# rslmtoasa/rslmtoasa

Measured on AMD Instinct MI355X. Metric: block-recursion throughput (H|psi> + A_n + B_n recursion levels, recursion.f90 recur_b), higher is better.
Workload: dtype f64

## Files before the change

### rslmtoasa_amd/csrc/kernels_mfma.hpp

```cpp
#pragma once
#include <hip/hip_runtime.h>
#include <string>
#include <vector>
#include "kernels_valu.hpp"

namespace rsrec {

typedef double double4_t __attribute__((ext_vector_type(4)));

constexpr int GROUP = 8;
constexpr int MF_WAVES = 4;

struct LayoutCI {
    static __device__ __forceinline__ double2 ld(const double* b, int r, int c) { return make_double2(b[36 * r + 2 * c], b[36 * r + 2 * c + 1]); }
    static __device__ __forceinline__ void st(double* b, int r, int c, double2 v) { b[36 * r + 2 * c] = v.x; b[36 * r + 2 * c + 1] = v.y; }
};
__host__ __device__ constexpr int gram_col(int part, int c, int ci) { return ci ? 2 * c + part : 18 * part + c; }

__device__ __forceinline__ int active_workgroups(int ngroups) { return max(1, min((int)gridDim.x, (ngroups + MF_WAVES - 1) / MF_WAVES)); }

struct GroupWalk {
    int g, end, step;
    __device__ __forceinline__ GroupWalk(int ngroups, int wave, int nbx_eff = 0) {
        const int nbx = nbx_eff > 0 ? nbx_eff : gridDim.x, bx = blockIdx.x;
        const int xcd = bx & 7, j = bx >> 3;
        const int per_xcd = (nbx >> 3) + ((xcd < (nbx & 7)) ? 1 : 0);
        const int chunk = (ngroups + 7) >> 3;
        const int lo = xcd * chunk;
        end = min(ngroups, lo + chunk);
        g = lo + j * MF_WAVES + wave;
        step = per_xcd * MF_WAVES;
        if (nbx < 8) { g = bx * MF_WAVES + wave; end = ngroups; step = nbx * MF_WAVES; }
    }
};


struct RowRef { unsigned off; bool valid; };
__device__ __forceinline__ RowRef group_row(const int* __restrict__ grp, int rho, int zero_block) {
    const int slot = rho / 18, r = rho - 18 * slot;
    const int a = grp[slot];
    RowRef R;
    R.valid = a >= 0;
    R.off = (unsigned)BLD * (unsigned)(R.valid ? a : zero_block) + 36u * (unsigned)r;
    return R;
}

struct GramAcc {
    double4_t t00, t01, t10, t11;
    double tr0, tr1;
    double t0r, t1r;
    double trr;
    __device__ __forceinline__ void zero() { t00 = t01 = t10 = t11 = (double4_t){0, 0, 0, 0}; tr0 = tr1 = t0r = t1r = trr = 0.0; }
    __device__ __forceinline__ void to_lds(double* G , int lane, bool sym) const {
        const int l15 = lane & 15, l4 = lane >> 4, l3 = lane & 3, lg = (lane >> 2) & 3;
#pragma unroll
        for (int j = 0; j < 4; ++j) {
            const int r = l4 + 4 * j;
            G[36 * r + l15] = t00[j];
            G[36 * r + 16 + l15] = t01[j];
            G[36 * (16 + r) + 16 + l15] = t11[j];
            if (!sym) G[36 * (16 + r) + l15] = t10[j];
        }
        G[36 * (32 + l4) + l15] = tr0;
        G[36 * (32 + l4) + 16 + l15] = tr1;
        if (!sym) { G[36 * (4 * lg + l4) + 32 + l3] = t0r; G[36 * (16 + 4 * lg + l4) + 32 + l3] = t1r; }
        if (lg == 0) G[36 * (32 + l4) + 32 + l3] = trr;
    }
};

__device__ __forceinline__ void gram_block_out(const GramAcc& A, double* lds , double* gout , bool sym) {
    const int lane = threadIdx.x & 63, wave = threadIdx.x >> 6;
    A.to_lds(lds + wave * 1296, lane, sym);
    __syncthreads();
    for (int e = threadIdx.x; e < 1296; e += blockDim.x) {
        double s = 0.0;
#pragma unroll
        for (int wv = 0; wv < MF_WAVES; ++wv) s += lds[wv * 1296 + e];
        if (sym) {
            const int r = e / 36, c = e % 36;
            const bool have = (r >= 32) || (r < 16) || (c >= 16 && c < 32);
            if (!have || (r < 32 && c >= 32)) {
                double t = 0.0;
#pragma unroll
                for (int wv = 0; wv < MF_WAVES; ++wv) t += lds[wv * 1296 + 36 * c + r];
                s = t;
            }
        }
        gout[e] = s;
    }
}

#ifndef RSREC_NT_STREAMS
#define RSREC_NT_STREAMS 0
#endif
template <class T> __device__ __forceinline__ T ld_stream(const T* p) {
#if RSREC_NT_STREAMS
    return __builtin_nontemporal_load(p);
#else
    return *p;
#endif
}
__device__ __forceinline__ double2 ld_stream(const double2* p) {
#if RSREC_NT_STREAMS
    typedef double nt_d2 __attribute__((ext_vector_type(2)));
    const nt_d2 v = __builtin_nontemporal_load(reinterpret_cast<const nt_d2*>(p));
    return make_double2(v[0], v[1]);
#else
    return *p;
#endif
}
template <class T> __device__ __forceinline__ void st_stream(T* p, T v) {
#if RSREC_NT_STREAMS
    __builtin_nontemporal_store(v, p);
#else
    *p = v;
#endif
}

constexpr int S5_GRAM_DOUBLES = 584;
constexpr long S5_GRAM_MIN_NEVER = 1L << 40;
constexpr int S5_GRAM_MAXW = 8;
__host__ __device__ inline bool s5_gram_folds(long ngroups, long min_groups) { return ngroups > 0 && ngroups >= min_groups; }
__host__ __device__ inline int s5_gram_workgroups(int ngroups) { return ngroups / 4 < 1 ? 1 : (ngroups / 4 < S5_GRAM_MAXW ? ngroups / 4 : S5_GRAM_MAXW); }
struct GramFold { const int* cum = nullptr; int nlev = 0; long min_groups = 0; };

__global__ __launch_bounds__(640) void k_gram_groupsum(GramFold F, int level, const double* __restrict__ gpart, size_t cstride, double* __restrict__ partial ) {
    __shared__ double sm[S5_GRAM_DOUBLES];
    const int chain = blockIdx.y, w = blockIdx.x;
    const int ngroups = F.cum[(size_t)chain * F.nlev + level] / GROUP;
    if (!s5_gram_folds(ngroups, F.min_groups)) return;
    double* img = partial + ((size_t)chain * gridDim.x + w) * 1296;
    const int nw = s5_gram_workgroups(ngroups);
    if (w >= nw) {
        for (int e = threadIdx.x; e < 1296; e += blockDim.x) img[e] = 0.0;
        return;
    }
    const size_t g0 = (size_t)w * ngroups / nw, g1 = (size_t)(w + 1) * ngroups / nw;
    if (threadIdx.x < S5_GRAM_DOUBLES) {
        const double* src = gpart + (size_t)chain * cstride + threadIdx.x;
        double s = 0.0;
        size_t q = 2 * g0;
        for (; q + 16 <= 2 * g1; q += 16) {
            double v[16];
#pragma unroll
            for (int i = 0; i < 16; ++i) v[i] = ld_stream(src + (q + i) * S5_GRAM_DOUBLES);
#pragma unroll
            for (int i = 0; i < 16; ++i) s += v[i];
        }
        for (; q < 2 * g1; ++q) s += ld_stream(src + q * S5_GRAM_DOUBLES);
        sm[threadIdx.x] = s;
    }
    __syncthreads();
    for (int e = threadIdx.x; e < 1296; e += blockDim.x) {
        const int r = e / 36, c = e - 36 * r, a = r >> 1, b = c >> 1, part = c & 1;
        double v = 0.0;
        if ((r & 1) == 0) {
            if (a < 16 && b < 16) v = sm[256 * part + 4 * (16 * (a & 3) + b) + (a >> 2)];
            else if (a >= 16 && b < 16) v = sm[512 + 2 * (16 * (a - 16) + b) + part];
            else if (a >= 16) v = sm[576 + 2 * (2 * (a - 16) + (b - 16)) + part];
            else { const double t = sm[512 + 2 * (16 * (b - 16) + a) + part]; v = part ? -t : t; }
        }
        img[e] = v;
    }
}

#ifndef ADOT_UNROLL
#define ADOT_UNROLL 4
#endif
__global__ __launch_bounds__(MF_WAVES * 64, 2) void k_mfma_adot(ChainView CV, int level, int zero_block, const double* __restrict__ psi,
                                                               const double* __restrict__ tvec, double* partial ,
                                                               GramFold F = GramFold() ) {
    __shared__ double lds[MF_WAVES * 1296];
    const int chain = blockIdx.y;
    if (F.cum && s5_gram_folds(F.cum[(size_t)chain * F.nlev + level] / GROUP, F.min_groups)) return;
    const int lane = threadIdx.x & 63;
    const int wave = __builtin_amdgcn_readfirstlane(threadIdx.x >> 6);
    const int ngroups = CV.count_of(chain, level) / GROUP;
    const int* order = CV.order_of(chain, level);
    const size_t vo = (size_t)chain * CV.vstride;
    const double* ps = psi + vo;
    const double* tv = tvec + vo;
    const int l15 = lane & 15, l4 = lane >> 4, l3 = lane & 3;
    GramAcc A;
    A.zero();
    const int nbx = active_workgroups(ngroups);
    for (GroupWalk w((int)blockIdx.x < nbx ? ngroups : 0, wave, nbx); w.g < w.end; w.g += w.step) {
        const int* grp = order + (size_t)w.g * GROUP;
#pragma unroll ADOT_UNROLL
        for (int kq = 0; kq < 36; ++kq) {
            const RowRef rk = group_row(grp, 4 * kq + l4, zero_block);
            const double p0 = ld_stream(ps + rk.off + l15), p1 = ld_stream(ps + rk.off + 16 + l15), pr = ld_stream(ps + rk.off + 32 + l3);
            const double h0 = ld_stream(tv + rk.off + l15), h1 = ld_stream(tv + rk.off + 16 + l15), hr = ld_stream(tv + rk.off + 32 + l3);
            A.t00 = __builtin_amdgcn_mfma_f64_16x16x4f64(p0, h0, A.t00, 0, 0, 0);
            A.t01 = __builtin_amdgcn_mfma_f64_16x16x4f64(p0, h1, A.t01, 0, 0, 0);
            A.t10 = __builtin_amdgcn_mfma_f64_16x16x4f64(p1, h0, A.t10, 0, 0, 0);
            A.t11 = __builtin_amdgcn_mfma_f64_16x16x4f64(p1, h1, A.t11, 0, 0, 0);
            A.tr0 = __builtin_amdgcn_mfma_f64_4x4x4f64(pr, h0, A.tr0, 0, 0, 0);
            A.tr1 = __builtin_amdgcn_mfma_f64_4x4x4f64(pr, h1, A.tr1, 0, 0, 0);
            A.t0r = __builtin_amdgcn_mfma_f64_4x4x4f64(p0, hr, A.t0r, 0, 0, 0);
            A.t1r = __builtin_amdgcn_mfma_f64_4x4x4f64(p1, hr, A.t1r, 0, 0, 0);
            A.trr = __builtin_amdgcn_mfma_f64_4x4x4f64(pr, hr, A.trr, 0, 0, 0);
        }
    }
    gram_block_out(A, lds, partial + ((size_t)chain * gridDim.x + blockIdx.x) * 1296, false);
}

struct SpmmDims {
    int kk, nslots, nmax, nlev, cpo, ostride, level; size_t vstride; const int* obase; int nchains = 0;
    int sat_base = 0, run_lo = 0, run_hi = 0, nskip = 0, skip_lo[4] = {0, 0, 0, 0}, skip_hi[4] = {0, 0, 0, 0};
    int nruns = 0, run_tau[4] = {0, 0, 0, 0}, run_glo[4] = {0, 0, 0, 0}, run_ghi[4] = {0, 0, 0, 0}, run_row0[5] = {0, 0, 0, 0, 0};
    int skip_pa = 0;
};

__device__ __forceinline__ double2 reduce_gram(const double* __restrict__ partial , int nblk, double* lds , int ci = 0) {
    for (int e = threadIdx.x; e < 1296; e += blockDim.x) {
        double s = 0.0;
        for (int p = 0; p < nblk; ++p) s += partial[(size_t)p * 1296 + e];
        lds[e] = s;
    }
    __syncthreads();
    double2 c = make_double2(0, 0);
    if (threadIdx.x < BLK) {
        const int cp = threadIdx.x % NB, cc = threadIdx.x / NB;
        const int rp = gram_col(0, cp, ci), ip = gram_col(1, cp, ci), rc = gram_col(0, cc, ci), ic = gram_col(1, cc, ci);
        c.x = lds[36 * rp + rc] + lds[36 * ip + ic];
        c.y = lds[36 * rp + ic] - lds[36 * ip + rc];
    }
    __syncthreads();
    return c;
}

}
```

### rslmtoasa_amd/csrc/kernels_spmm5.hpp

```cpp
#pragma once
#include <hip/hip_runtime.h>
#include <algorithm>
#include <type_traits>
#include <utility>
#include <vector>
#include "kernels_valu.hpp"
#include "kernels_mfma.hpp"
#include "kernels_spmm4.hpp"

namespace rsrec {

#ifndef RSREC_S5_KSPLIT_PROBE
#define RSREC_S5_KSPLIT_PROBE 0
#endif
#ifndef RSREC_S5_PRIO
#define RSREC_S5_PRIO 0
#endif
#ifndef RSREC_S5_GRAM_STRIP_LOADS
#define RSREC_S5_GRAM_STRIP_LOADS 0
#endif
#ifndef S5_WG_GROUPS
#define S5_WG_GROUPS 4
#endif
constexpr int S5_TRIPLE = 640;
// ... 744 lines not shown
                        ecr[i] = cb[eo[i] + 288 + (l4 & 1)];
                    }
                    if (epi.kind == 2) {
                        const double* zb = epi.old + vo;
#pragma unroll
                        for (int i = 0; i < 3; ++i) {
#pragma unroll
                            for (int p = 0; p < 2; ++p) ez[i][p] = *reinterpret_cast<const s5_d2*>(zb + eo[i] + 36 * (4 * p + l4));
                            ezr[i] = zb[eo[i] + 288 + (l4 & 1)];
                        }
                    }
                }
#pragma unroll
                for (int i = 0; i < 3; ++i) {
                    const int a = av[i];
                    double* ob = out + eo[i];
#pragma unroll
                    for (int p = 0; p < 2; ++p) {
                        s5_d2 v; v[0] = acc3.m[i][2 * p]; v[1] = acc3.m[i][2 * p + 1];
                        if (epi.kind) {
                            v[0] = (v[0] - epi.b * ec[i][p][0]) / epi.a; v[1] = (v[1] - epi.b * ec[i][p][1]) / epi.a;
                            if (epi.kind == 2) { v[0] = v[0] * 2.0 - ez[i][p][0]; v[1] = v[1] * 2.0 - ez[i][p][1]; }
                        }
                        if (a != zero_block) *reinterpret_cast<s5_d2*>(ob + 36 * (4 * p + l4)) = v;
                    }
                    double r = acc3.r[i];
                    if (epi.kind) {
                        r = (r - epi.b * ecr[i]) / epi.a;
                        if (epi.kind == 2) r = r * 2.0 - ezr[i];
                    }
                    if (a != zero_block && l4 < 2) ob[288 + l4] = r;
                }
            };
            int ratom[GROUP];
            if (part < 2) {
                int a3[3];
#pragma unroll
                for (int j = 0; j < 3; ++j) { const int a = grp[3 * part + j]; a3[j] = a >= 0 ? a : zero_block; }
#pragma unroll
                for (int t = 0; t < GROUP; ++t) ratom[t] = zero_block;
                s5_run_stream_n<TWO, 3, false>(acc3, M3, fr3, inb, in2b, nbr, a3, ratom, 0, ncol, sig, l4, lane_main, lane_z, lane_rem, lane_rem_z, lane16, lane8);
                finish3(std::false_type{}, a3);
            } else {
#pragma unroll
                for (int t = 0; t < GROUP; ++t) { const int a = grp[t]; ratom[t] = a >= 0 ? a : zero_block; }
                const int a2[2] = {ratom[6], ratom[7]};
                int mra = grp[l15 >> 1];
                mra = mra >= 0 ? mra : zero_block;
                s5_run_stream_n<TWO, 2, true>(acc3, M3, fr3, inb, in2b, nbr, a2, ratom, l15 >> 1, ncol, sig, l4, lane_main, lane_z, lane_rem, lane_rem_z, lane16, lane8);
                const int av[3] = {a2[0], a2[1], mra};
                finish3(std::true_type{}, av);
            }
            continue;
        }
        int atom[GROUP];
        int vatom[GROUP], tile_blk[GROUP];
        int my_rem_atom, rem_blk = 0;
        if constexpr (OCT) {
            const int a0 = g;
#pragma unroll
            for (int t = 0; t < GROUP; ++t) {
                const bool ok = a0 >= 0 && chain + t < D.nchains;
                atom[t] = ok ? a0 : zero_block;
                tile_blk[t] = ok ? t * (D.kk + 1) : 0;
                vatom[t] = ok ? a0 + t * (D.kk + 1) : zero_block;
            }
            const int tr = l15 >> 1;
            const bool okr = a0 >= 0 && chain + tr < D.nchains;
            rem_blk = okr ? tr * (D.kk + 1) : 0;
            my_rem_atom = okr ? a0 + tr * (D.kk + 1) : zero_block;
        } else {
#pragma unroll
            for (int t = 0; t < GROUP; ++t) { const int a = grp[t]; atom[t] = a >= 0 ? a : zero_block; vatom[t] = atom[t]; tile_blk[t] = 0; }
            my_rem_atom = grp[l15 >> 1];
            my_rem_atom = my_rem_atom >= 0 ? my_rem_atom : zero_block;
        }
        const int first = atom[0];
        if (!OCT && D.skip_pa && first < D.nmax) continue;
        const int tau = first < D.nmax ? first : D.nmax + izp[first];
        const int* __restrict__ M = meta + (size_t)tau * Spmm5Operator::META;
        const char* __restrict__ fr = LDSA ? reinterpret_cast<const char*>(s5_lds) : reinterpret_cast<const char*>(frag + ((size_t)tau * 2 + sig) * ntr * S5_TRIPLE);
        const char* __restrict__ fh = (TWO && frag_head) ? reinterpret_cast<const char*>(frag_head + ((size_t)chain * ntau + tau) * S5_HEAD_DOUBLES + (size_t)sig * S5_HEAD_TRIPLES * S5_TRIPLE) : nullptr;

        S5Acc acc;
#pragma unroll
        for (int t = 0; t < 9; ++t) { acc.m[t] = (double4_t){0, 0, 0, 0}; acc.r[t] = 0.0; }

        if constexpr (OCT) s5_run_stream<TWO, LDSA, true>(acc, M, fr, fh, inb, in2b, nbr, atom, l15 >> 1, ncol, sig, l4, lane_main, lane_z, lane_rem, lane_rem_z, lane16, lane8, tile_blk, rem_blk);
        else s5_run_stream<TWO, LDSA>(acc, M, fr, fh, inb, in2b, nbr, atom, l15 >> 1, ncol, sig, l4, lane_main, lane_z, lane_rem, lane_rem_z, lane16, lane8, tile_blk, rem_blk, kpart);
#if RSREC_S5_KSPLIT_PROBE
        if (kpart) continue;
#endif

        int fl15 = l15, fl4 = l4;
        if constexpr (GRAM) {
            unsigned fl;
            asm volatile("v_mbcnt_lo_u32_b32 %0, -1, 0\n\tv_mbcnt_hi_u32_b32 %0, -1, %0" : "=v"(fl));
            fl15 = (int)fl & 15; fl4 = (int)fl >> 4;
        }
        const int ekind = GRAM ? 0 : epi.kind;
        auto finish = [&](auto t0c, auto t1c) {
            constexpr int T0 = decltype(t0c)::value, T1 = decltype(t1c)::value, NT = T1 - T0;
            size_t eo[NT];
#pragma unroll
            for (int i = 0; i < NT; ++i) { const int t = T0 + i; eo[i] = (size_t)BLD * ((t < 8) ? vatom[t] : my_rem_atom) + 324 * sig + ((t < 8) ? 2 * fl15 : 32 + 2 * (fl15 & 1)); }
            s5_d2 ec[NT][2], ez[NT][2];
            double ecr[NT], ezr[NT];
            if (ekind) {
                const double* cb = epi.cur + vo;
#pragma unroll
                for (int i = 0; i < NT; ++i) {
#pragma unroll
                    for (int p = 0; p < 2; ++p) ec[i][p] = *reinterpret_cast<const s5_d2*>(cb + eo[i] + 36 * (4 * p + fl4));
                    ecr[i] = cb[eo[i] + 288 + (fl4 & 1)];
                }
                if (ekind == 2) {
                    const double* zb = epi.old + vo;
#pragma unroll
                    for (int i = 0; i < NT; ++i) {
#pragma unroll
                        for (int p = 0; p < 2; ++p) ez[i][p] = *reinterpret_cast<const s5_d2*>(zb + eo[i] + 36 * (4 * p + fl4));
                        ezr[i] = zb[eo[i] + 288 + (fl4 & 1)];
                    }
                }
            }
#pragma unroll
            for (int i = 0; i < NT; ++i) {
                const int t = T0 + i;
                const int a = (t < 8) ? vatom[t] : my_rem_atom;
                double* ob = out + eo[i];
#pragma unroll
                for (int p = 0; p < 2; ++p) {
                    s5_d2 v; v[0] = acc.m[t][2 * p]; v[1] = acc.m[t][2 * p + 1];
                    if (ekind) {
                        v[0] = (v[0] - epi.b * ec[i][p][0]) / epi.a; v[1] = (v[1] - epi.b * ec[i][p][1]) / epi.a;
                        if (ekind == 2) { v[0] = v[0] * 2.0 - ez[i][p][0]; v[1] = v[1] * 2.0 - ez[i][p][1]; }
                    }
                    if (a != zero_block) *reinterpret_cast<s5_d2*>(ob + 36 * (4 * p + fl4)) = v;
                }
                double r = acc.r[t];
                if (ekind) {
                    r = (r - epi.b * ecr[i]) / epi.a;
                    if (ekind == 2) r = r * 2.0 - ezr[i];
                }
                if (a != zero_block && fl4 < 2) ob[288 + fl4] = r;
            }
        };
        bool stored = false;
        if constexpr (GRAM) if (fold) {
            unsigned gl;
            asm volatile("v_mbcnt_lo_u32_b32 %0, -1, 0\n\tv_mbcnt_hi_u32_b32 %0, -1, %0" : "=v"(gl));
            const int lane = (int)gl, l15 = lane & 15, l4 = lane >> 4;
            const double* __restrict__ ub = in_all + vo;
            double4_t gre = {0, 0, 0, 0}, gim = {0, 0, 0, 0};
            double sre[2] = {0.0, 0.0}, sim[2] = {0.0, 0.0}, kre[2] = {0.0, 0.0}, kim[2] = {0.0, 0.0};
            auto rem_coef = [&](s5_d2 u, double& cr, double& ci) {
                cr = l4 == 0 ? u[0] : (l4 == 1 ? u[1] : 0.0);
                ci = l4 == 0 ? -u[1] : (l4 == 1 ? u[0] : 0.0);
            };
            constexpr bool STRIP_LOADS = RSREC_S5_GRAM_STRIP_LOADS != 0;
            auto strip_loads = [&](s5_d2 (&gs)[3][2], const double* ab) {
#pragma unroll
                for (int p = 0; p < 3; ++p)
#pragma unroll
                    for (int e = 0; e < 2; ++e) gs[p][e] = *reinterpret_cast<const s5_d2*>(ab + 36 * (p < 2 ? 4 * p + l4 : 8) + 32 + 2 * e);
            };
            s5_d2 gs8[3][2];
            if constexpr (!STRIP_LOADS) strip_loads(gs8, ub + (size_t)BLD * my_rem_atom + 324 * sig);
            auto gram_tiles = [&](auto t0c, auto t1c) {
                constexpr int T0 = decltype(t0c)::value, T1 = decltype(t1c)::value, NT = T1 - T0;
                s5_d2 gu[NT][3], gs[STRIP_LOADS ? NT : 1][3][2];
#pragma unroll
                for (int i = 0; i < NT; ++i) {
                    const int t = T0 + i;
                    const double* ab = ub + (size_t)BLD * ((t < 8) ? vatom[t] : my_rem_atom) + 324 * sig;
#pragma unroll
                    for (int p = 0; p < 3; ++p)
                        if (t < 8) gu[i][p] = *reinterpret_cast<const s5_d2*>(ab + 36 * (p < 2 ? 4 * p + l4 : 8) + 2 * l15);
                    if constexpr (STRIP_LOADS) strip_loads(gs[i], ab);
                }
                if constexpr (!STRIP_LOADS && T0 == 0) {
                    __builtin_amdgcn_sched_barrier(0);
                    finish(S5C<0>{}, S5C<5>{});
                    finish(S5C<5>{}, S5C<9>{});
                    stored = true;
                    __builtin_amdgcn_sched_barrier(0);
                }
                s5_each_tile<T0>(std::make_integer_sequence<int, NT>{}, [&](auto tc, auto ic) {
                    constexpr int t = decltype(tc)::value, i = decltype(ic)::value;
                    const double x8 = acc.r[t];
                    if constexpr (t < 8) {
#pragma unroll
                        for (int p = 0; p < 2; ++p) {
                            gre = __builtin_amdgcn_mfma_f64_16x16x4f64(gu[i][p][0], acc.m[t][2 * p], gre, 0, 0, 0);
                            gre = __builtin_amdgcn_mfma_f64_16x16x4f64(gu[i][p][1], acc.m[t][2 * p + 1], gre, 0, 0, 0);
                            gim = __builtin_amdgcn_mfma_f64_16x16x4f64(-gu[i][p][1], acc.m[t][2 * p], gim, 0, 0, 0);
                            gim = __builtin_amdgcn_mfma_f64_16x16x4f64(gu[i][p][0], acc.m[t][2 * p + 1], gim, 0, 0, 0);
                        }
                        double cr, ci;
                        rem_coef(gu[i][2], cr, ci);
                        gre = __builtin_amdgcn_mfma_f64_16x16x4f64(cr, x8, gre, 0, 0, 0);
                        gim = __builtin_amdgcn_mfma_f64_16x16x4f64(ci, x8, gim, 0, 0, 0);
                    }
                    auto strip = [&](int p, int e) -> s5_d2 {
                        if constexpr (STRIP_LOADS) return gs[i][p][e];
                        else if constexpr (t < 8) return s5_row_bcast<2 * t>(gs8[p][e]);
                        else return gs8[p][e];
                    };
                    double (&are)[2] = (t < 8) ? sre : kre;
                    double (&aim)[2] = (t < 8) ? sim : kim;
#pragma unroll
                    for (int e = 0; e < 2; ++e) {
#pragma unroll
                        for (int p = 0; p < 2; ++p) {
                            const s5_d2 u = strip(p, e);
                            const double ur = u[0], ui = u[1], tr = acc.m[t][2 * p], ti = acc.m[t][2 * p + 1];
                            are[e] = fma(ur, tr, are[e]); are[e] = fma(ui, ti, are[e]);
                            aim[e] = fma(ur, ti, aim[e]); aim[e] = fma(-ui, tr, aim[e]);
                        }
                        double cr, ci;
                        rem_coef(strip(2, e), cr, ci);
                        are[e] = fma(cr, x8, are[e]);
                        aim[e] = fma(ci, x8, aim[e]);
                    }
                });
                if constexpr (!STRIP_LOADS) {
                    if constexpr (T0 < 8) asm volatile("" : "+v"(sre[0]), "+v"(sre[1]), "+v"(sim[0]), "+v"(sim[1]));
                    if constexpr (T1 == 9) asm volatile("" : "+v"(kre[0]), "+v"(kre[1]), "+v"(kim[0]), "+v"(kim[1]));
                }
            };
            if constexpr (STRIP_LOADS) {
                gram_tiles(S5C<0>{}, S5C<2>{});
                __builtin_amdgcn_sched_barrier(0);
                gram_tiles(S5C<2>{}, S5C<4>{});
                __builtin_amdgcn_sched_barrier(0);
                gram_tiles(S5C<4>{}, S5C<6>{});
                __builtin_amdgcn_sched_barrier(0);
                gram_tiles(S5C<6>{}, S5C<8>{});
                __builtin_amdgcn_sched_barrier(0);
                gram_tiles(S5C<8>{}, S5C<9>{});
            } else {
                gram_tiles(S5C<0>{}, S5C<4>{});
                __builtin_amdgcn_sched_barrier(0);
                gram_tiles(S5C<4>{}, S5C<9>{});
            }
            __builtin_amdgcn_sched_barrier(0);
            auto sum_l4 = [&](double v) {
                double s = __shfl(v, l15);
                s += __shfl(v, l15 + 16); s += __shfl(v, l15 + 32); s += __shfl(v, l15 + 48);
                return s;
            };
            auto sum_atoms = [&](double v) {
                double s = __shfl(v, l15 & 1);
#pragma unroll
                for (int a = 1; a < GROUP; ++a) s += __shfl(v, 2 * a + (l15 & 1));
                return s;
            };
            double* gp = gram.out + (size_t)chain * gram.cstride + ((size_t)g * 2 + sig) * S5_GRAM_DOUBLES;
            s5_d2 v;
#pragma unroll
            for (int p = 0; p < 2; ++p) {
                v[0] = gre[2 * p]; v[1] = gre[2 * p + 1];
                *reinterpret_cast<s5_d2*>(gp + 4 * lane + 2 * p) = v;
                v[0] = gim[2 * p]; v[1] = gim[2 * p + 1];
                *reinterpret_cast<s5_d2*>(gp + 256 + 4 * lane + 2 * p) = v;
            }
#pragma unroll
            for (int e = 0; e < 2; ++e) {
                v[0] = sum_l4(sre[e]); v[1] = sum_l4(sim[e]);
                if (l4 == e) *reinterpret_cast<s5_d2*>(gp + 512 + 2 * (16 * e + l15)) = v;
                v[0] = sum_atoms(sum_l4(kre[e])); v[1] = sum_atoms(sum_l4(kim[e]));
                if (lane < 2) *reinterpret_cast<s5_d2*>(gp + 576 + 2 * (2 * e + lane)) = v;
            }
        }
        if (!stored) {
            finish(S5C<0>{}, S5C<5>{});
            finish(S5C<5>{}, S5C<9>{});
        }
    }
    }
}

}
```

### rslmtoasa_amd/csrc/rsrec.hip

```cpp
#include <hip/hip_runtime.h>
#include <hsa/hsa.h>
#include <hsa/hsa_ext_amd.h>
#include <dlfcn.h>
#include <algorithm>
#include <array>
#include <atomic>
#include <chrono>
#include <cmath>
#include <cstdarg>
#include <cstdio>
#include <cstdlib>
#include <cstring>
#include <memory>
#include <string>
#include <thread>
#include <tuple>
#include <vector>

#include "../../include/rsrec.h"
#include "kernels_valu.hpp"
#include "kernels_mfma.hpp"
#include "kernels_spmm4.hpp"
#include "kernels_spmm5.hpp"
#include "kernels_uscheme.hpp"
// ... 1396 lines not shown
    double a, b;
    int level = 0;
    ChainChebyshev(const rsrec_t* h, const RecursionCall& RC, double a_, double b_)
        : old(h->d_vec[1].as<double>()), cur(h->d_vec[0].as<double>()), spare(h->d_vec[2].as<double>()), tmp(h->d_vec[3].as<double>()),
          hps(RC.ci && h->hoh ? h->d_vec[4].as<double>() : nullptr), a(a_), b(b_) {}
    int step(rsrec_t* h, RecursionCall& RC, const RecursionBatch& bt, int t, bool plain_h = false) {
        const bool first = t == 1;
        if (first) std::swap(old, cur);
        else { double* o = spare; spare = old; old = cur; cur = o; }
        level = h->hoh ? 2 * t : t;
        if (RC.mfma) return apply_h(h, RC, bt, t, old, plain_h ? tmp : cur, hps, nullptr, 0, plain_h ? S5Epilogue() : cheb_epilogue(first, old, spare, a, b));
        if (first) return valu_apply_h<AM_CHEB1, AM_HOH_CHEB1>(h, RC, bt, t, old, old, cur, tmp, a, b);
        return valu_apply_h<AM_CHEBN, AM_HOH_CHEBN>(h, RC, bt, t, old, spare, cur, tmp, a, b);
    }
};

template <class Pass>
int chain_level_loop(rsrec_t* h, RecursionCall& RC, const RecursionBatch& bt, double a, double b, Pass&& pass) {
    XFER(clear_vectors(h, RC, bt.nb));
    ChainChebyshev S(h, RC, a, b);
    seed_chains(h, RC, bt.nb, S.cur);
    pass(S.cur, 0, 0);
    for (int t = 1; t <= RC.napply; ++t) {
        XFER(S.step(h, RC, bt, t));
        pass(S.cur, S.level, t);
    }
    HIPCK(h, hipGetLastError());
    HIPCK(h, hipStreamSynchronize(h->stream));
    return RSREC_OK;
}
struct SideReduce { bool side = false, pending = false; };
int side_reduce_begin(rsrec_t* h, const SideReduce& S, hipStream_t& st) {
    st = S.side ? h->side_stream : h->stream;
    if (S.side) { HIPCK(h, hipEventRecord(h->ev_orth, h->stream)); HIPCK(h, hipStreamWaitEvent(h->side_stream, h->ev_orth, 0)); }
    return RSREC_OK;
}
int side_reduce_end(rsrec_t* h, SideReduce& S) { if (S.side) { HIPCK(h, hipEventRecord(h->ev_bred, h->side_stream)); S.pending = true; } return RSREC_OK; }
int side_reduce_wait(rsrec_t* h, SideReduce& S) { if (S.pending) { HIPCK(h, hipStreamWaitEvent(h->stream, h->ev_bred, 0)); S.pending = false; } return RSREC_OK; }

template <class Enqueue>
int replay_level_loop(rsrec_t* h, const std::vector<uintptr_t>& key, Enqueue&& enqueue) {
    if (!h->graph_exec || key != h->graph_key) {
        if (h->graph_exec) { (void)hipGraphExecDestroy(h->graph_exec); h->graph_exec = nullptr; }
        h->graph_key.clear();
        s5_prepare(h);
        XFER(s4_prepare(h));
        HIPCK(h, hipStreamSynchronize(h->stream));
        HIPCK(h, hipStreamBeginCapture(h->stream, hipStreamCaptureModeRelaxed));
        h->capturing = true;
        const int rc = enqueue();
        h->capturing = false;
        hipGraph_t graph = nullptr;
        const hipError_t ec = hipStreamEndCapture(h->stream, &graph);
        if (rc) { if (graph) (void)hipGraphDestroy(graph); return rc; }
        if (ec != hipSuccess || !graph) return fail(h, RSREC_ERR_DEVICE, "hipStreamEndCapture failed: %s", hipGetErrorString(ec));
        const hipError_t ei = hipGraphInstantiate(&h->graph_exec, graph, nullptr, nullptr, 0);
        (void)hipGraphDestroy(graph);
        if (ei != hipSuccess) { h->graph_exec = nullptr; return fail(h, RSREC_ERR_DEVICE, "hipGraphInstantiate failed: %s", hipGetErrorString(ei)); }
        h->graph_key = key;
    }
    HIPCK(h, hipGraphLaunch(h->graph_exec, h->stream));
    return RSREC_OK;
}

int rotate_resident_coef(rsrec_t* h, RecursionCall& RC, double2* dA, double2* dB, int c0, int nb, int lld) {
    hipEvent_t r0 = next_event(h);
    k_rotate_coef<<<dim3(2 * (lld - 1), nb), 256, 0, h->stream>>>(dA, dB, h->d_rot.as<double2>() + (size_t)c0 * BLK, lld);
    HIPCK(h, hipGetLastError());
    RC.rot_ev.emplace_back(r0, next_event(h));
    return RSREC_OK;
}
int recursion_end(rsrec_t* h, const RecursionCall& RC, int res_kind, int lld, bool seeded) {
    hipEvent_t ev_end = next_event(h);
    const int rc = finish_status(h);
    finish_timing(h, RC.ev_begin, ev_end, RC.hop_ev);
    for (auto& pr : RC.rot_ev) h->t_rot_ms += ev_ms(pr.first, pr.second);
    if (rc) return rc;
    h->res_kind = res_kind; h->res_n = RC.nchains; h->res_lld = lld; h->res_seeded = seeded;
    return RSREC_OK;
}

template <class L, bool MFMA>
int run_block_lanczos(rsrec_t* h, int nchains, int nseed, const int32_t* seed_atoms, const double* seed_coef, int lld, double* a_b, double* b2_b,
                      const double* rot = nullptr ) {
    const int kk = h->kk;
    const bool hoh = h->hoh != 0;
    const int nsteps = lld - 1;
    if (rot && !MFMA) return fail(h, RSREC_ERR_ARG, "local-axis recursion needs the matrix-core kernel set (option kernels = 0 or 2)");
    RecursionCall RC = recursion_call(h, MFMA, nchains, nseed, nsteps, rot);
    const int ci = RC.ci, ntau = h->nmax + h->ntype;
    const size_t cstride = (size_t)lld * BLK, orth_lds = TILE_ATOMS * BLK * sizeof(double2);
    drop_resident(h);
    HIPCK(h, h->d_coefA.reserve((size_t)nchains * lld * BLK * sizeof(double2)));
    HIPCK(h, h->d_coefB.reserve((size_t)nchains * lld * BLK * sizeof(double2)));
    if (rot) {
        HIPCK(h, h->d_rot.reserve((size_t)nchains * BLK * sizeof(double2)));
        XFER(xfer_h2d(h, h->d_rot.p, rot, (size_t)nchains * BLK * sizeof(double2)));
    }
    const bool oop = MFMA && h->opt_orth_oop != 0 && h->opt_orth3 != 2;
    const int nvec = MFMA ? (oop && hoh ? 5 : 4) : (hoh ? 3 : 2);
    const bool use_v1 = !MFMA || hoh || oop;
    const size_t gram_groups = ((size_t)kk + 7 * (size_t)(h->nmax + h->ntype) + 8 + GROUP - 1) / GROUP;
    const bool gram_eligible = MFMA && ci && !hoh && !rot && h->ntype == 1 && h->nmax == 0 && h->ham_hermitian && h->opt_s5_split != 3 &&
                               RC.op->single_class(0) >= 0 && (h->opt_nblk <= 0 || 2 * h->opt_nblk >= S5_GRAM_MAXW) &&
                               s5_gram_folds((long)gram_groups, h->opt_s5_gram_min);
    const size_t gram_cstride = gram_eligible ? gram_groups * 2 * S5_GRAM_DOUBLES : 0;
    XFER(recursion_begin(h, RC, nvec, use_v1 ? -1 : 1, nseed, gram_cstride));
    const int B = RC.B, nblk = RC.nblk;
    HIPCK(h, h->d_frags.reserve((size_t)B * 3 * 27 * 64 * sizeof(double)));
    HIPCK(h, h->d_bmats.reserve((size_t)B * 2 * BLK * sizeof(double2)));
    const size_t gram_elems = (size_t)B * 256 * 1296;
    double *pmn = h->d_vec[1].as<double>(), *hpsi = h->d_vec[2].as<double>();
    double2* partial = h->d_partial.as<double2>();
    double *gpartial = h->d_partial.as<double>(), *bfrags = h->d_frags.as<double>();
    HIPCK(h, hipFuncSetAttribute(reinterpret_cast<const void*>(k_orth<L>), hipFuncAttributeMaxDynamicSharedMemorySize, TILE_ATOMS * BLK * (int)sizeof(double2)));
    h->hop_fuses_a = MFMA ? 0 : 1;

    for (int c0 = 0; c0 < nchains; c0 += B) {
        const int nb = std::min(B, nchains - c0);
        double2* dA = h->d_coefA.as<double2>() + (size_t)c0 * cstride;
        double2* dB = h->d_coefB.as<double2>() + (size_t)c0 * cstride;
        RecursionBatch bt;
        XFER(recursion_batch(h, RC, seed_atoms, seed_coef, c0, nb, bt));
        const ChainView &CV = bt.CV, &CVp = bt.CVp;
        const rsrec_handle::RegionEntry* RE = h->cur_entry;
        auto fold_at = [&](int lv) -> int {
            if (!gram_eligible || !RE || lv < 0 || lv >= (int)RE->hop_max.size()) return 0;
            if (!s5_gram_folds(RE->hop_max[lv] / GROUP, h->opt_s5_gram_min)) return 0;
            return s5_gram_folds(RE->hop_min[lv] / GROUP, h->opt_s5_gram_min) ? 2 : 1;
        };
        for (int ll = 0; ll < nsteps; ++ll) { const int f = fold_at(ll + 1); h->n_gram_folded += f > 0; h->n_gram_all += f == 2; h->n_gram_levels += 1; }
        auto enqueue_levels = [&]() -> int {
            XFER(clear_vectors(h, RC, nb, MFMA && !hoh ? 2 : -1));
            HIPCK(h, hipMemsetAsync(dA, 0, (size_t)nb * cstride * sizeof(double2), h->stream));
            HIPCK(h, hipMemsetAsync(dB, 0, (size_t)nb * cstride * sizeof(double2), h->stream));
            if (MFMA) HIPCK(h, hipMemsetAsync(bfrags, 0, (size_t)nb * 3 * 27 * 64 * sizeof(double), h->stream));
            double *psi = h->d_vec[0].as<double>(), *t2 = h->d_vec[3].as<double>();
            double* t3 = oop ? h->d_vec[hoh ? 4 : 1].as<double>() : nullptr;
            seed_chains(h, RC, nb, psi);
            k_set_identity<<<nb, 256, 0, h->stream>>>(dB, cstride);
            if (MFMA) k_uscheme_init<<<nb, 256, 0, h->stream>>>(h->d_bmats.as<double2>(), bfrags, ci);
            const dim3 grid(nblk, nb);
            SideReduce SR{RC.side};
            double* gp_b = SR.side ? gpartial + gram_elems : gpartial;
            for (int ll = 0; ll < nsteps; ++ll) {
                const int lv_final = hoh ? 2 * ll + 2 : ll + 1;
                if (MFMA) {
                    const int folds = fold_at(lv_final);
                    const GramFold GF{folds ? CV.cum : nullptr, RC.nlev, h->opt_s5_gram_min};
                    XFER(apply_h(h, RC, bt, ll + 1, psi, hpsi, pmn, bt.la_extra, ntau, S5Epilogue(),
                                 folds ? S5Gram{h->d_gram.as<double>(), gram_cstride, h->opt_s5_gram_min} : S5Gram()));
                    const dim3 gl = level_grid(h, bt.grid_mf, lv_final);
                    if (folds < 2) k_mfma_adot<<<gl, MF_WAVES * 64, 0, h->stream>>>(CVp, lv_final, kk, psi, hpsi, gpartial, GF);
                    if (folds) k_gram_groupsum<<<gl, 640, 0, h->stream>>>(GF, lv_final, h->d_gram.as<double>(), gram_cstride, gpartial);
                    int n2 = gl.x; const double* p2 = presum(h, gpartial, nb, n2, 1296);
                    XFER(side_reduce_wait(h, SR));
                    k_reduce_a_u<<<nb, 1024, 0, h->stream>>>(p2, n2, dA + (size_t)ll * BLK, cstride, h->d_bmats.as<double2>(), bfrags, ci);
                    if (h->opt_orth3 == 2) k_mfma_orth3w<<<gl, MF_WAVES * 64, 0, h->stream>>>(CVp, lv_final, kk, hpsi, psi, t2, bfrags, gp_b);
                    else k_mfma_orth3<<<gl, MF_WAVES * 64, 0, h->stream>>>(CVp, lv_final, kk, hpsi, psi, t2, bfrags, gp_b, t3);
                    hipStream_t st; XFER(side_reduce_begin(h, SR, st));
                    n2 = gl.x; p2 = presum(h, gp_b, nb, n2, 1296, st, SR.side ? 1 : 0);
                    k_reduce_b_u<<<nb, 1024, 0, st>>>(p2, n2, dB + (size_t)(ll + 1) * BLK, cstride, h->d_bmats.as<double2>(), bfrags, h->d_status.as<int>(), ci);
                    XFER(side_reduce_end(h, SR));
                    if (oop) { double* f = t2; t2 = psi; psi = t3; t3 = f; }
                    else std::swap(psi, t2);
                    continue;
                }
                XFER((valu_apply_h<AM_LANCZOS, AM_HOH_LANCZOS>(h, RC, bt, ll + 1, psi, psi, pmn, hpsi)));
                k_reduce_a<<<nb, 1024, 0, h->stream>>>(partial, nblk, dA + (size_t)ll * BLK, cstride);
                k_orth<L><<<grid, NTHREADS, orth_lds, h->stream>>>(CV, lv_final, psi, pmn, (const double*)nullptr, dA + (size_t)ll * BLK, cstride, partial);
                k_reduce_b_eig<<<nb, 1024, 0, h->stream>>>(partial, nblk, dB + (size_t)(ll + 1) * BLK, cstride, h->d_bmats.as<double2>(), h->d_status.as<int>());
                k_update<L><<<grid, NTHREADS, 0, h->stream>>>(CV, lv_final, psi, pmn, h->d_bmats.as<double2>());
            }
            HIPCK(h, hipGetLastError());
            return side_reduce_wait(h, SR);
        };
        const bool use_graph = MFMA && nchains <= B && ((h->opt_graph == 1 && nchains <= 8) || h->opt_graph >= 2) && getenv("RSREC_NO_GRAPH") == nullptr;
        if (!use_graph) XFER(enqueue_levels());
        else {
            if (ci) HIPCK(h, h->d_s5queue.reserve((size_t)nb * 16 * sizeof(int)));
            const Spmm5Operator& OP = *RC.op;
            std::vector<uintptr_t> key = {(uintptr_t)1 , (uintptr_t)nb, (uintptr_t)lld, (uintptr_t)nseed, (uintptr_t)hoh, (uintptr_t)ci, (uintptr_t)(rot != nullptr), (uintptr_t)kk,
                                          (uintptr_t)h->cur_order, (uintptr_t)h->cur_cum, (uintptr_t)bt.ostride, (uintptr_t)OP.d_frag, (uintptr_t)OP.d_meta, (uintptr_t)OP.ntr,
                                          (uintptr_t)h->s4_op.frag_set(0), (uintptr_t)h->s4_op.meta_set(0), (uintptr_t)h->d_nbr.p, (uintptr_t)h->d_nbr5.p, (uintptr_t)h->d_iz.p,
                                          (uintptr_t)h->d_partial.p, (uintptr_t)h->d_partial2.p, (uintptr_t)h->d_frags.p, (uintptr_t)dA, (uintptr_t)dB, (uintptr_t)h->d_bmats.p,
                                          (uintptr_t)h->d_status.p, (uintptr_t)h->d_seed.p, (uintptr_t)h->d_seedcoef.p, (uintptr_t)h->d_la_extra.p, (uintptr_t)h->d_s5queue.p,
                                          (uintptr_t)h->cur_entry, (uintptr_t)h->p2_slot, (uintptr_t)OP.single_class(0), (uintptr_t)OP.spin_mixing,
                                          (uintptr_t)h->lattice_epoch, (uintptr_t)OP.sched_epoch, (uintptr_t)h->nslots, (uintptr_t)h->nmax, (uintptr_t)h->ntype, (uintptr_t)h->hslots,
                                          (uintptr_t)B, (uintptr_t)h->n_cu, (uintptr_t)h->d_gram.p, (uintptr_t)gram_eligible};
            for (int v = 0; v < nvec; ++v) key.push_back((uintptr_t)h->d_vec[v].p);
            for (const OptionEntry& o : OPTIONS)
                if (o.member != &rsrec_handle::opt_graph) key.push_back((uintptr_t)(h->*o.member));
            XFER(replay_level_loop(h, key, enqueue_levels));
            h->n_hop_launch += (double)nsteps * (hoh ? 2 : 1);
        }
        if (rot && lld > 1) XFER(rotate_resident_coef(h, RC, dA, dB, c0, nb, lld));
        XFER(xfer_d2h(h, a_b + (size_t)c0 * cstride * 2, dA, (size_t)nb * cstride * sizeof(double2)));
        XFER(xfer_d2h(h, b2_b + (size_t)c0 * cstride * 2, dB, (size_t)nb * cstride * sizeof(double2)));
        HIPCK(h, hipStreamSynchronize(h->stream));
    }
    if (MFMA && h->n_gram_levels > 0 && h->n_gram_all == h->n_gram_levels) h->hop_fuses_a = 1;
    return recursion_end(h, RC, 1, lld, seed_coef != nullptr);
}

}

extern "C" int rsrec_block_lanczos_seeded(rsrec_t* h, int nchains, int nseed, const int32_t* seed_atoms, const double* seed_coef, int lld,
                                          double* a_b, double* b2_b) {
    int rc = check_ready(h, "rsrec_block_lanczos");
    if (rc) return rc;
    if (nchains < 0 || nseed < 1 || lld < 1 || !a_b || !b2_b || (nchains > 0 && !seed_atoms)) return fail(h, RSREC_ERR_ARG, "rsrec_block_lanczos: bad argument");
    XFER(check_seeds(h, "rsrec_block_lanczos", seed_atoms, (size_t)nchains * nseed, 1));
    HIPCK(h, hipSetDevice(h->device));
    reset_timing(h);
    if (nchains == 0) return RSREC_OK;
    if (matrix_core_set(h)) return run_block_lanczos<LayoutRM, true>(h, nchains, nseed, seed_atoms, seed_coef, lld, a_b, b2_b);
    return run_block_lanczos<LayoutCM, false>(h, nchains, nseed, seed_atoms, seed_coef, lld, a_b, b2_b);
}

extern "C" int rsrec_block_lanczos(rsrec_t* h, int nsites, const int32_t* seed_atoms, int lld, double* a_b, double* b2_b) {
    return rsrec_block_lanczos_seeded(h, nsites, 1, seed_atoms, nullptr, lld, a_b, b2_b);
}

namespace {

int build_local_axis_operator(rsrec_t* h) {
    if (h->s5_la_ok) return RSREC_OK;
    const int ntau = h->nmax + h->ntype, nfs = h->nslots + 1, nset = h->hoh ? 2 : 1;
    const size_t B = 2 * (size_t)BLK;
    std::vector<const double*> blk((size_t)nset * ntau * nfs, nullptr);
    std::vector<double> dense(B, 1.0), neg((size_t)ntau * h->nslots * B, 0.0);
    for (int tau = 0; tau < ntau; ++tau) {
        for (int s = 0; s < h->nslots; ++s) {
            const double* src = tau < h->nmax ? h->host_hall.data() + B * (s + (size_t)h->hslots * tau) : h->host_ee.data() + B * (s + (size_t)h->hslots * (tau - h->nmax));
            blk[((size_t)0 * ntau + tau) * nfs + s] = src;
            if (nset > 1) {
                const double* so = tau < h->nmax ? h->host_hallo.data() + B * (s + (size_t)h->hslots * tau) : h->host_eeo.data() + B * (s + (size_t)h->hslots * (tau - h->nmax));
                double* d = neg.data() + B * (s + (size_t)h->nslots * tau);
                for (size_t e = 0; e < B; ++e) d[e] = -so[e];
                if (s == 0) for (int q = 0; q < NB; ++q) d[2 * (q + NB * q)] += 1.0;
                blk[((size_t)1 * ntau + tau) * nfs + s] = d;
            }
        }
        blk[((size_t)(nset - 1) * ntau + tau) * nfs + h->nslots] = dense.data();
    }
    const char* msg = h->s5_la.build_custom(h->nslots, ntau, nset, blk);
    if (msg) return fail(h, RSREC_ERR_DEVICE, "rsrec_block_lanczos_local_axis: %s", msg);
    h->s5_la_ok = 1;
    return RSREC_OK;
}

}

extern "C" int rsrec_block_lanczos_local_axis(rsrec_t* h, int nsites, const int32_t* seed_atoms, const double* rot, int lld, double* a_b, double* b2_b) {
    int rc = check_ready(h, "rsrec_block_lanczos_local_axis");
    if (rc) return rc;
    if (nsites < 0 || lld < 1 || !a_b || !b2_b || (nsites > 0 && (!seed_atoms || !rot))) return fail(h, RSREC_ERR_ARG, "rsrec_block_lanczos_local_axis: bad argument");
    XFER(check_seeds(h, "rsrec_block_lanczos_local_axis", seed_atoms, (size_t)nsites, 1));
    if (!h->s5_built) return fail(h, RSREC_ERR_ARG, "rsrec_block_lanczos_local_axis: lattice has too many neighbour slots for the SpMM kernel");
    HIPCK(h, hipSetDevice(h->device));
    reset_timing(h);
    if (nsites == 0) return RSREC_OK;
    rc = build_local_axis_operator(h); if (rc) return rc;
    return run_block_lanczos<LayoutRM, true>(h, nsites, 1, seed_atoms, nullptr, lld, a_b, b2_b, rot);
}

namespace {

bool is_device_ptr(const void* p) {
    hipPointerAttribute_t at;
    if (hipPointerGetAttributes(&at, p) == hipSuccess) return at.type == hipMemoryTypeDevice;
    (void)hipGetLastError();
    hsa_amd_pointer_info_t info;
    memset(&info, 0, sizeof info);
    info.size = sizeof info;
    if (hsa_amd_pointer_info(const_cast<void*>(p), &info, nullptr, nullptr, nullptr) != HSA_STATUS_SUCCESS) return false;
    if (info.type != HSA_EXT_POINTER_TYPE_HSA) return false;
    hsa_device_type_t dt = HSA_DEVICE_TYPE_CPU;
    if (hsa_agent_get_info(info.agentOwner, HSA_AGENT_INFO_DEVICE, &dt) != HSA_STATUS_SUCCESS) return false;
    return dt == HSA_DEVICE_TYPE_GPU;
}

__global__ void k_pack_diag(const double2* __restrict__ A, const double2* __restrict__ B, int lld, int n, int off, int ntot,
                            double* __restrict__ a_img, double* __restrict__ b_img) {
    const size_t total = (size_t)lld * NB * ntot;
    for (size_t e = (size_t)blockIdx.x * blockDim.x + threadIdx.x; e < total; e += (size_t)gridDim.x * blockDim.x) {
        const int ll = (int)(e % lld), l = (int)((e / lld) % NB), s = (int)(e / ((size_t)lld * NB)) - off;
        double a = 0.0, b = 0.0;
        if (s >= 0 && s < n) {
            const size_t q = ((size_t)s * lld + ll) * BLK + (size_t)l * (NB + 1);
            a = A[q].x; b = B[q].x;
        }
        a_img[e] = a; b_img[e] = b;
    }
}

}

extern "C" int rsrec_pack_diag(rsrec_t* h, int site_offset, int nsites_total, double* a_img, double* b2_img) {
    if (!h || !a_img || !b2_img || site_offset < 0) return fail(h, RSREC_ERR_ARG, "rsrec_pack_diag: bad argument");
    if (h->res_kind != 1) return fail(h, RSREC_ERR_ARG, "rsrec_pack_diag: no block-Lanczos coefficients resident (call rsrec_block_lanczos first)");
    if (site_offset + h->res_n > nsites_total) return fail(h, RSREC_ERR_ARG, "rsrec_pack_diag: sites %d..%d outside 1..%d", site_offset + 1, site_offset + h->res_n, nsites_total);
    HIPCK(h, hipSetDevice(h->device));
    const size_t n = (size_t)h->res_lld * NB * nsites_total;
    const bool dev = is_device_ptr(a_img) && is_device_ptr(b2_img);
    double *da = a_img, *db = b2_img;
    if (!dev) { HIPCK(h, h->d_scal.reserve(2 * n * sizeof(double))); da = h->d_scal.as<double>(); db = da + n; }
// ... 2333 lines not shown
```

Before: 69490.

## Fold Gram real/imag MFMA accumulators into one using Hermitian symmetry

Replaces the separate real and imaginary 16x16 Gram accumulators in the fused SpMM epilogue with one accumulator fed by (re-im) and (re+im) combinations. The group-sum kernel then recovers the real and imaginary parts from the symmetric and antisymmetric halves (S_ab ± S_ba)/2. This halves the MFMA count and the per-group partial storage and streaming reads (584→328 doubles), and shrinks the groupsum block to 384 threads. It relies on the Gram block being Hermitian, and the recombination could change rounding slightly.

```diff
diff --git a/rslmtoasa_amd/csrc/kernels_mfma.hpp b/rslmtoasa_amd/csrc/kernels_mfma.hpp
--- a/rslmtoasa_amd/csrc/kernels_mfma.hpp
+++ b/rslmtoasa_amd/csrc/kernels_mfma.hpp
@@ -117,14 +117,14 @@
 #endif
 }
 
-constexpr int S5_GRAM_DOUBLES = 584;
+constexpr int S5_GRAM_DOUBLES = 328;
 constexpr long S5_GRAM_MIN_NEVER = 1L << 40;
 constexpr int S5_GRAM_MAXW = 8;
 __host__ __device__ inline bool s5_gram_folds(long ngroups, long min_groups) { return ngroups > 0 && ngroups >= min_groups; }
 __host__ __device__ inline int s5_gram_workgroups(int ngroups) { return ngroups / 4 < 1 ? 1 : (ngroups / 4 < S5_GRAM_MAXW ? ngroups / 4 : S5_GRAM_MAXW); }
 struct GramFold { const int* cum = nullptr; int nlev = 0; long min_groups = 0; };
 
-__global__ __launch_bounds__(640) void k_gram_groupsum(GramFold F, int level, const double* __restrict__ gpart, size_t cstride, double* __restrict__ partial ) {
+__global__ __launch_bounds__(384) void k_gram_groupsum(GramFold F, int level, const double* __restrict__ gpart, size_t cstride, double* __restrict__ partial ) {
     __shared__ double sm[S5_GRAM_DOUBLES];
     const int chain = blockIdx.y, w = blockIdx.x;
     const int ngroups = F.cum[(size_t)chain * F.nlev + level] / GROUP;
@@ -155,10 +155,13 @@
         const int r = e / 36, c = e - 36 * r, a = r >> 1, b = c >> 1, part = c & 1;
         double v = 0.0;
         if ((r & 1) == 0) {
-            if (a < 16 && b < 16) v = sm[256 * part + 4 * (16 * (a & 3) + b) + (a >> 2)];
-            else if (a >= 16 && b < 16) v = sm[512 + 2 * (16 * (a - 16) + b) + part];
-            else if (a >= 16) v = sm[576 + 2 * (2 * (a - 16) + (b - 16)) + part];
-            else { const double t = sm[512 + 2 * (16 * (b - 16) + a) + part]; v = part ? -t : t; }
+            if (a < 16 && b < 16) {
+                const double sab = sm[4 * (16 * (a & 3) + b) + (a >> 2)], sba = sm[4 * (16 * (b & 3) + a) + (b >> 2)];
+                v = 0.5 * (part ? sab - sba : sab + sba);
+            }
+            else if (a >= 16 && b < 16) v = sm[256 + 2 * (16 * (a - 16) + b) + part];
+            else if (a >= 16) v = sm[320 + 2 * (2 * (a - 16) + (b - 16)) + part];
+            else { const double t = sm[256 + 2 * (16 * (b - 16) + a) + part]; v = part ? -t : t; }
         }
         img[e] = v;
     }
diff --git a/rslmtoasa_amd/csrc/kernels_spmm5.hpp b/rslmtoasa_amd/csrc/kernels_spmm5.hpp
--- a/rslmtoasa_amd/csrc/kernels_spmm5.hpp
+++ b/rslmtoasa_amd/csrc/kernels_spmm5.hpp
@@ -920,24 +920,24 @@
             asm volatile("v_mbcnt_lo_u32_b32 %0, -1, 0\n\tv_mbcnt_hi_u32_b32 %0, -1, %0" : "=v"(gl));
             const int lane = (int)gl, l15 = lane & 15, l4 = lane >> 4;
             const double* __restrict__ ub = in_all + vo;
-            double4_t gre = {0, 0, 0, 0}, gim = {0, 0, 0, 0};
+            double4_t gs = {0, 0, 0, 0};
             double sre[2] = {0.0, 0.0}, sim[2] = {0.0, 0.0}, kre[2] = {0.0, 0.0}, kim[2] = {0.0, 0.0};
             auto rem_coef = [&](s5_d2 u, double& cr, double& ci) {
                 cr = l4 == 0 ? u[0] : (l4 == 1 ? u[1] : 0.0);
                 ci = l4 == 0 ? -u[1] : (l4 == 1 ? u[0] : 0.0);
             };
             constexpr bool STRIP_LOADS = RSREC_S5_GRAM_STRIP_LOADS != 0;
-            auto strip_loads = [&](s5_d2 (&gs)[3][2], const double* ab) {
+            auto strip_loads = [&](s5_d2 (&gst)[3][2], const double* ab) {
 #pragma unroll
                 for (int p = 0; p < 3; ++p)
 #pragma unroll
-                    for (int e = 0; e < 2; ++e) gs[p][e] = *reinterpret_cast<const s5_d2*>(ab + 36 * (p < 2 ? 4 * p + l4 : 8) + 32 + 2 * e);
+                    for (int e = 0; e < 2; ++e) gst[p][e] = *reinterpret_cast<const s5_d2*>(ab + 36 * (p < 2 ? 4 * p + l4 : 8) + 32 + 2 * e);
             };
             s5_d2 gs8[3][2];
             if constexpr (!STRIP_LOADS) strip_loads(gs8, ub + (size_t)BLD * my_rem_atom + 324 * sig);
             auto gram_tiles = [&](auto t0c, auto t1c) {
                 constexpr int T0 = decltype(t0c)::value, T1 = decltype(t1c)::value, NT = T1 - T0;
-                s5_d2 gu[NT][3], gs[STRIP_LOADS ? NT : 1][3][2];
+                s5_d2 gu[NT][3], gst[STRIP_LOADS ? NT : 1][3][2];
 #pragma unroll
                 for (int i = 0; i < NT; ++i) {
                     const int t = T0 + i;
@@ -945,7 +945,7 @@
 #pragma unroll
                     for (int p = 0; p < 3; ++p)
                         if (t < 8) gu[i][p] = *reinterpret_cast<const s5_d2*>(ab + 36 * (p < 2 ? 4 * p + l4 : 8) + 2 * l15);
-                    if constexpr (STRIP_LOADS) strip_loads(gs[i], ab);
+                    if constexpr (STRIP_LOADS) strip_loads(gst[i], ab);
                 }
                 if constexpr (!STRIP_LOADS && T0 == 0) {
                     __builtin_amdgcn_sched_barrier(0);
@@ -960,18 +960,16 @@
                     if constexpr (t < 8) {
 #pragma unroll
                         for (int p = 0; p < 2; ++p) {
-                            gre = __builtin_amdgcn_mfma_f64_16x16x4f64(gu[i][p][0], acc.m[t][2 * p], gre, 0, 0, 0);
-                            gre = __builtin_amdgcn_mfma_f64_16x16x4f64(gu[i][p][1], acc.m[t][2 * p + 1], gre, 0, 0, 0);
-                            gim = __builtin_amdgcn_mfma_f64_16x16x4f64(-gu[i][p][1], acc.m[t][2 * p], gim, 0, 0, 0);
-                            gim = __builtin_amdgcn_mfma_f64_16x16x4f64(gu[i][p][0], acc.m[t][2 * p + 1], gim, 0, 0, 0);
+                            const double um = gu[i][p][0] - gu[i][p][1], up = gu[i][p][0] + gu[i][p][1];
+                            gs = __builtin_amdgcn_mfma_f64_16x16x4f64(um, acc.m[t][2 * p], gs, 0, 0, 0);
+                            gs = __builtin_amdgcn_mfma_f64_16x16x4f64(up, acc.m[t][2 * p + 1], gs, 0, 0, 0);
                         }
                         double cr, ci;
                         rem_coef(gu[i][2], cr, ci);
-                        gre = __builtin_amdgcn_mfma_f64_16x16x4f64(cr, x8, gre, 0, 0, 0);
-                        gim = __builtin_amdgcn_mfma_f64_16x16x4f64(ci, x8, gim, 0, 0, 0);
+                        gs = __builtin_amdgcn_mfma_f64_16x16x4f64(cr + ci, x8, gs, 0, 0, 0);
                     }
                     auto strip = [&](int p, int e) -> s5_d2 {
-                        if constexpr (STRIP_LOADS) return gs[i][p][e];
+                        if constexpr (STRIP_LOADS) return gst[i][p][e];
                         else if constexpr (t < 8) return s5_row_bcast<2 * t>(gs8[p][e]);
                         else return gs8[p][e];
                     };
@@ -1028,17 +1026,15 @@
             s5_d2 v;
 #pragma unroll
             for (int p = 0; p < 2; ++p) {
-                v[0] = gre[2 * p]; v[1] = gre[2 * p + 1];
+                v[0] = gs[2 * p]; v[1] = gs[2 * p + 1];
                 *reinterpret_cast<s5_d2*>(gp + 4 * lane + 2 * p) = v;
-                v[0] = gim[2 * p]; v[1] = gim[2 * p + 1];
-                *reinterpret_cast<s5_d2*>(gp + 256 + 4 * lane + 2 * p) = v;
             }
 #pragma unroll
             for (int e = 0; e < 2; ++e) {
                 v[0] = sum_l4(sre[e]); v[1] = sum_l4(sim[e]);
-                if (l4 == e) *reinterpret_cast<s5_d2*>(gp + 512 + 2 * (16 * e + l15)) = v;
+                if (l4 == e) *reinterpret_cast<s5_d2*>(gp + 256 + 2 * (16 * e + l15)) = v;
                 v[0] = sum_atoms(sum_l4(kre[e])); v[1] = sum_atoms(sum_l4(kim[e]));
-                if (lane < 2) *reinterpret_cast<s5_d2*>(gp + 576 + 2 * (2 * e + lane)) = v;
+                if (lane < 2) *reinterpret_cast<s5_d2*>(gp + 320 + 2 * (2 * e + lane)) = v;
             }
         }
         if (!stored) {
diff --git a/rslmtoasa_amd/csrc/rsrec.hip b/rslmtoasa_amd/csrc/rsrec.hip
--- a/rslmtoasa_amd/csrc/rsrec.hip
+++ b/rslmtoasa_amd/csrc/rsrec.hip
@@ -1572,7 +1572,7 @@
                                  folds ? S5Gram{h->d_gram.as<double>(), gram_cstride, h->opt_s5_gram_min} : S5Gram()));
                     const dim3 gl = level_grid(h, bt.grid_mf, lv_final);
                     if (folds < 2) k_mfma_adot<<<gl, MF_WAVES * 64, 0, h->stream>>>(CVp, lv_final, kk, psi, hpsi, gpartial, GF);
-                    if (folds) k_gram_groupsum<<<gl, 640, 0, h->stream>>>(GF, lv_final, h->d_gram.as<double>(), gram_cstride, gpartial);
+                    if (folds) k_gram_groupsum<<<gl, 384, 0, h->stream>>>(GF, lv_final, h->d_gram.as<double>(), gram_cstride, gpartial);
                     int n2 = gl.x; const double* p2 = presum(h, gpartial, nb, n2, 1296);
                     XFER(side_reduce_wait(h, SR));
                     k_reduce_a_u<<<nb, 1024, 0, h->stream>>>(p2, n2, dA + (size_t)ll * BLK, cstride, h->d_bmats.as<double2>(), bfrags, ci);
```

Result: faster. 71550, median of 6 (+3.0%).
